# Scalsol/mega.pytorch

Measured on AMD Instinct MI355X. Metric: frames/sec MEGA R-101 inference, 1000x600 VID clip, higher is better.
Workload: dtype bf16

## Files before the change

### mega/pytorch_amd/csrc/spatial.hip

```cpp
#include <cstdlib>

#include "common.h"

namespace {

constexpr int ST_T = 16;
constexpr int ST_P = ST_T * 2 + 5;
constexpr int ST_PW = ST_P + 1;

template <typename OT>
__global__ __launch_bounds__(256) void stem_conv_kernel(const float* __restrict__ in, const float* __restrict__ w,
                                                        const float* __restrict__ scale,
                                                        const float* __restrict__ bias, OT* __restrict__ out, int N,
                                                        int H, int W, int Ho, int Wo) {
  __shared__ float patch[3][ST_P][ST_PW];
  const int tid = threadIdx.x;
  const int n = blockIdx.z;
  const int oy0 = blockIdx.y * ST_T, ox0 = blockIdx.x * ST_T;
  const int iy0 = oy0 * 2 - 3, ix0 = ox0 * 2 - 3;
  for (int e = tid; e < 3 * ST_P * ST_P; e += 256) {
    const int c = e / (ST_P * ST_P);
    const int rem = e - c * ST_P * ST_P;
    const int y = rem / ST_P, x = rem - y * ST_P;
    const int iy = iy0 + y, ix = ix0 + x;
// ... 268 lines not shown
  constexpr int VE = Elem<T>::VE;
  int xo[NC];
#pragma unroll
  for (int c = 0; c < NC; ++c) xo[c] = min(x0 + c, W - 1) * C;
  for (int r = 0; r < NR; r += RU) {
    uint4 rv[RU][NC];
#pragma unroll
    for (int u = 0; u < RU; ++u) {
      const T* rowp = base + (size_t)min(y0 + r + u, H - 1) * W * C;
#pragma unroll
      for (int c = 0; c < NC; ++c) rv[u][c] = *reinterpret_cast<const uint4*>(rowp + xo[c]);
    }
#pragma unroll
    for (int u = 0; u < RU; ++u) {
      const float wyr = r + u < RS_MAXP ? wy[r + u] : 0.f;
#pragma unroll
      for (int c = 0; c < NC; ++c) {
        const T* ev = reinterpret_cast<const T*>(&rv[u][c]);
        const float wgt = wyr * wx[c];
#pragma unroll
        for (int e = 0; e < VE; ++e) acc[e] = fmaf(wgt, Elem<T>::ld(ev + e), acc[e]);
      }
    }
  }
}

template <typename T, int NSLICE, bool PLANES = false, typename PT = bf16_t>
__global__ __launch_bounds__(256, 4) void roi_align_nhwc_sep_kernel(const T* __restrict__ feat,
                                                                 const float* __restrict__ rois, T* __restrict__ out,
                                                                 int K, int C, int H, int W, float spatial_scale,
                                                                 int PH, int PW) {
  static_assert(!PLANES || sizeof(T) == 4, "planes output: f32 features");
  constexpr int VE = Elem<T>::VE;
  auto store = [&](int k_, int bin, int cv, const float (&acc)[Elem<T>::VE], float inv_count) {
    if constexpr (PLANES) {
      float v[4];
#pragma unroll
      for (int e = 0; e < 4; ++e) v[e] = acc[e] * inv_count;
      const unsigned h0 = Half16<PT>::pack2(v[0], v[1]), h1 = Half16<PT>::pack2(v[2], v[3]);
      const unsigned l0 = Half16<PT>::pack2(v[0] - Half16<PT>::lo(h0), v[1] - Half16<PT>::hi(h0));
      const unsigned l1 = Half16<PT>::pack2(v[2] - Half16<PT>::lo(h1), v[3] - Half16<PT>::hi(h1));
      const size_t plane = (size_t)PH * PW * C;
      unsigned short* row = reinterpret_cast<unsigned short*>(out) + (size_t)k_ * 2 * plane + (size_t)bin * C + (size_t)cv * 4;
      *reinterpret_cast<uint2*>(row) = make_uint2(h0, h1);
      *reinterpret_cast<uint2*>(row + plane) = make_uint2(l0, l1);
    } else {
      uint4 o;
      T* oe = reinterpret_cast<T*>(&o);
#pragma unroll
      for (int e = 0; e < VE; ++e) Elem<T>::st(oe + e, acc[e] * inv_count);
      *reinterpret_cast<uint4*>(out + ((size_t)k_ * PH * PW + bin) * C + (size_t)cv * VE) = o;
    }
  };
  __shared__ float s_wy[RS_MAXPW][RS_MAXP + 2];
  __shared__ float s_wx[RS_MAXPW][RS_MAXP];
  __shared__ int s_y[RS_MAXPW][2];
  __shared__ int s_x[RS_MAXPW][2];
  const int CV = C / VE;
  const int slice = NSLICE == 8 ? (int)(blockIdx.x & 7) : 0;
  const int k = NSLICE == 8 ? (int)(blockIdx.x >> 3) : (int)blockIdx.x;
  const int cvs = CV / NSLICE;
  const float* roi = rois + (size_t)k * 5;
  const int b = (int)roi[0];
  const float roi_start_w = roi[1] * spatial_scale;
  const float roi_start_h = roi[2] * spatial_scale;
  const float roi_end_w = roi[3] * spatial_scale;
  const float roi_end_h = roi[4] * spatial_scale;
  const float roi_width = fmaxf(roi_end_w - roi_start_w, 1.f);
  const float roi_height = fmaxf(roi_end_h - roi_start_h, 1.f);
  const float bin_size_h = roi_height / (float)PH;
  const float bin_size_w = roi_width / (float)PW;
  const int grid_h = (int)ceilf(roi_height / (float)PH);
  const int grid_w = (int)ceilf(roi_width / (float)PW);
  const float count = (float)(grid_h * grid_w);
  auto axis = [](float p, int n, int& lo, int& hi, float& wl, float& wh) {
    if (p < -1.0f || p > (float)n) { lo = hi = 0; wl = wh = 0.f; return; }
    if (p <= 0.f) p = 0.f;
    lo = (int)p;
    if (lo >= n - 1) { hi = lo = n - 1; p = (float)lo; } else { hi = lo + 1; }
    wh = p - (float)lo;
    wl = 1.f - wh;
  };
  auto table = [&](float start, float bin_size, int bin_index, int grid, int n, int slot, int& first, int& cnt) {
    int f = n, l = -1;
    for (int i = 0; i < grid; ++i) {
      int lo, hi; float wl, wh;
      axis(start + bin_index * bin_size + (i + .5f) * bin_size / (float)grid, n, lo, hi, wl, wh);
      if (wl + wh > 0.f) { f = min(f, lo); l = max(l, hi); }
    }
    float w = 0.f;
    for (int i = 0; i < grid; ++i) {
      int lo, hi; float wl, wh;
      axis(start + bin_index * bin_size + (i + .5f) * bin_size / (float)grid, n, lo, hi, wl, wh);
      if (wl + wh > 0.f) {
        if (lo - f == slot) w += wl;
        if (hi - f == slot) w += wh;
      }
    }
    if (l < f) { f = 0; l = -1; }
    first = f;
    cnt = l - f + 1;
    return w;
  };
  const int tid = threadIdx.x;
  if (tid < PH * (RS_MAXP + 2)) {
    const int ph = tid / (RS_MAXP + 2), slot = tid - ph * (RS_MAXP + 2);
    int first, cnt;
    const float w = table(roi_start_h, bin_size_h, ph, grid_h, H, slot, first, cnt);
    s_wy[ph][slot] = slot < RS_MAXP ? w : 0.f;
    if (slot == 0) { s_y[ph][0] = first; s_y[ph][1] = cnt; }
  } else if (tid >= 128 && tid < 128 + PW * RS_MAXP) {
    const int pw = (tid - 128) / RS_MAXP, slot = (tid - 128) - pw * RS_MAXP;
    int first, cnt;
    s_wx[pw][slot] = table(roi_start_w, bin_size_w, pw, grid_w, W, slot, first, cnt);
    if (slot == 0) { s_x[pw][0] = first; s_x[pw][1] = cnt; }
  }
  __syncthreads();
  int NR = 0, NCm = 0;
  for (int i = 0; i < PH; ++i) NR = max(NR, s_y[i][1]);
  for (int i = 0; i < PW; ++i) NCm = max(NCm, s_x[i][1]);
  const float inv_count = 1.f / count;
  const T* fb = feat + (size_t)b * H * W * C;
  const int nitem = PH * PW * cvs;
  if (NR > RS_MAXP || NCm > RS_MAXP) {
    for (int item = tid; item < nitem; item += 256) {
      const int bin = item / cvs, ph = bin / PW, pw = bin - ph * PW;
      const int cv = slice * cvs + (item - bin * cvs);
      float acc[VE];
#pragma unroll
      for (int e = 0; e < VE; ++e) acc[e] = 0.f;
      for (int iy = 0; iy < grid_h; ++iy) {
        int ylo, yhi; float wyl, wyh;
        axis(roi_start_h + ph * bin_size_h + (iy + .5f) * bin_size_h / (float)grid_h, H, ylo, yhi, wyl, wyh);
        for (int ix = 0; ix < grid_w; ++ix) {
          int xlo, xhi; float wxl, wxh;
          axis(roi_start_w + pw * bin_size_w + (ix + .5f) * bin_size_w / (float)grid_w, W, xlo, xhi, wxl, wxh);
          if (wyl + wyh == 0.f || wxl + wxh == 0.f) continue;
          const int ys[2] = {ylo, yhi}, xs[2] = {xlo, xhi};
          const float wys[2] = {wyl, wyh}, wxs[2] = {wxl, wxh};
#pragma unroll
          for (int a = 0; a < 2; ++a)
#pragma unroll
            for (int c = 0; c < 2; ++c) {
              const uint4 v = *reinterpret_cast<const uint4*>(fb + ((size_t)ys[a] * W + xs[c]) * C + (size_t)cv * VE);
              const T* ev = reinterpret_cast<const T*>(&v);
              const float wgt = wys[a] * wxs[c];
#pragma unroll
              for (int e = 0; e < VE; ++e) acc[e] = fmaf(wgt, Elem<T>::ld(ev + e), acc[e]);
            }
        }
      }
      store(k, bin, cv, acc, inv_count);
    }
    return;
  }
  for (int item = tid; item < nitem; item += 256) {
    const int bin = item / cvs, ph = bin / PW, pw = bin - ph * PW;
    const int cv = slice * cvs + (item - bin * cvs);
    float acc[VE];
#pragma unroll
    for (int e = 0; e < VE; ++e) acc[e] = 0.f;
    const T* base = fb + (size_t)cv * VE;
    const int y0 = s_y[ph][0], x0 = s_x[pw][0];
    if (NCm <= 3) roi_patch_accumulate<T, 3, 2>(base, W, H, C, y0, x0, NR, s_wy[ph], s_wx[pw], acc);
    else if (NCm <= 4) roi_patch_accumulate<T, 4, 2>(base, W, H, C, y0, x0, NR, s_wy[ph], s_wx[pw], acc);
    else if (NCm <= 6) roi_patch_accumulate<T, 6, 2>(base, W, H, C, y0, x0, NR, s_wy[ph], s_wx[pw], acc);
    else roi_patch_accumulate<T, RS_MAXP, 1>(base, W, H, C, y0, x0, NR, s_wy[ph], s_wx[pw], acc);
    store(k, bin, cv, acc, inv_count);
  }
}

constexpr int SM_TY = 8, SM_TX = 32;
constexpr int SM_PH = 2 * SM_TY + 5, SM_PW = 2 * SM_TX + 5, SM_PS = 72;
constexpr int SM_K = 176, SM_WS = 184;

__host__ __device__ constexpr int stem_group_off(int g) {
  const int gg = g < 21 ? g : 20;
  return (gg / 7) * (SM_PH * SM_PS) + (gg % 7) * SM_PS;
}

template <bool U8>
__global__ __launch_bounds__(256, 4) void stem_mfma_kernel(const void* __restrict__ in_, const bf16_t* __restrict__ w,
                                                        const float* __restrict__ scale,
                                                        const float* __restrict__ bias, bf16_t* __restrict__ out,
                                                        int N, int H, int W, int Ho, int Wo, float m0, float m1, float m2,
                                                        int to_bgr) {
  const float* __restrict__ in = reinterpret_cast<const float*>(in_);
  const unsigned char* __restrict__ in8 = reinterpret_cast<const unsigned char*>(in_);
  constexpr int SM_PATCH_B = (3 * SM_PH * SM_PS * 2 + 15) / 16 * 16, SM_OUT_PS = 144;
  constexpr int SM_LDS_B = SM_TY * SM_TX * SM_OUT_PS > SM_PATCH_B + 64 * SM_WS * 2 ? SM_TY * SM_TX * SM_OUT_PS
                                                                                   : SM_PATCH_B + 64 * SM_WS * 2;
  __shared__ __attribute__((aligned(16))) unsigned char smem[SM_LDS_B];
  unsigned short* patch = reinterpret_cast<unsigned short*>(smem);
  unsigned short* wl = reinterpret_cast<unsigned short*>(smem + SM_PATCH_B);
  const int tid = threadIdx.x, lane = tid & 63, wave = tid >> 6;
  const int n = blockIdx.z;
  const int oy0 = blockIdx.y * SM_TY, ox0 = blockIdx.x * SM_TX;
  const int iy0 = oy0 * 2 - 3, ix0 = ox0 * 2 - 3;
  constexpr int NPL = (3 * SM_PH * SM_PS + 255) / 256, NWL = (64 * (SM_K / 8) + 255) / 256;
  float pv[NPL];
  u32x4_t wv[NWL];
#pragma unroll
  for (int i = 0; i < NPL; ++i) {
    const int e = tid + 256 * i;
    const int c = e / (SM_PH * SM_PS);
    const int rem = e - c * (SM_PH * SM_PS);
    const int y = rem / SM_PS, x = rem - y * SM_PS;
    const int iy = iy0 + y, ix = ix0 + x;
    pv[i] = 0.f;
    if (e < 3 * SM_PH * SM_PS && x < SM_PW && (unsigned)iy < (unsigned)H && (unsigned)ix < (unsigned)W) {
      if (U8) {
        const float mean = c == 0 ? m0 : (c == 1 ? m1 : m2);
        pv[i] = (float)in8[(((size_t)n * H + iy) * W + ix) * 3 + (to_bgr ? 2 - c : c)] - mean;
      } else {
        pv[i] = in[((size_t)(n * 3 + c) * H + iy) * W + ix];
      }
    }
  }
#pragma unroll
  for (int i = 0; i < NWL; ++i) {
    const int e = tid + 256 * i;
    const int row = e / (SM_K / 8), v = e - row * (SM_K / 8);
    if (e < 64 * (SM_K / 8)) wv[i] = *reinterpret_cast<const u32x4_t*>(w + row * SM_K + v * 8);
  }
#pragma unroll
  for (int i = 0; i < NPL; ++i) {
    const int e = tid + 256 * i;
    if (e < 3 * SM_PH * SM_PS) patch[e] = f32_to_bf16(pv[i]);
  }
#pragma unroll
  for (int i = 0; i < NWL; ++i) {
    const int e = tid + 256 * i;
    const int row = e / (SM_K / 8), v = e - row * (SM_K / 8);
    if (e < 64 * (SM_K / 8)) *reinterpret_cast<u32x4_t*>(&wl[row * SM_WS + v * 8]) = wv[i];
  }
  __syncthreads();

  const int p = lane & 31, half = lane >> 5;
  f32x16_t acc[2][2];
#pragma unroll
  for (int i = 0; i < 2; ++i)
#pragma unroll
    for (int j = 0; j < 2; ++j)
#pragma unroll
      for (int r = 0; r < 16; ++r) acc[i][j][r] = 0.f;
#pragma unroll
  for (int ks = 0; ks < SM_K / 16; ++ks) {
    uint4 a[2], b[2];
#pragma unroll
    for (int i = 0; i < 2; ++i) {
      const unsigned* base = reinterpret_cast<const unsigned*>(
          patch + (2 * (2 * wave + i)) * SM_PS + 2 * p + (half ? stem_group_off(2 * ks + 1) : stem_group_off(2 * ks)));
      a[i] = make_uint4(base[0], base[1], base[2], base[3]);
    }
#pragma unroll
    for (int j = 0; j < 2; ++j)
      b[j] = *reinterpret_cast<const uint4*>(&wl[(j * 32 + p) * SM_WS + ks * 16 + half * 8]);
#pragma unroll
    for (int i = 0; i < 2; ++i)
#pragma unroll
      for (int j = 0; j < 2; ++j)
        acc[i][j] = __builtin_amdgcn_mfma_f32_32x32x16_bf16(__builtin_bit_cast(bf16x8_t, a[i]),
                                                            __builtin_bit_cast(bf16x8_t, b[j]), acc[i][j], 0, 0, 0);
  }
  __syncthreads();
#pragma unroll
  for (int j = 0; j < 2; ++j) {
    const int ch = j * 32 + p;
    const float sc = scale[ch], bi = bias[ch];
#pragma unroll
    for (int i = 0; i < 2; ++i) {
#pragma unroll
      for (int r = 0; r < 16; ++r) {
        const int px = (r & 3) + 8 * (r >> 2) + 4 * half;
        *reinterpret_cast<unsigned short*>(smem + ((2 * wave + i) * SM_TX + px) * SM_OUT_PS + ch * 2) =
            (bf16_t)(f32_to_bf16(fmaxf(acc[i][j][r] * sc + bi, 0.f)) & 0x7fffu);
      }
    }
  }
  __syncthreads();
#pragma unroll
  for (int i = 0; i < SM_TY * SM_TX * 8 / 256; ++i) {
    const int v = tid + 256 * i;
    const int pl = v >> 3, cv = v & 7;
    const int oy = oy0 + pl / SM_TX, ox = ox0 + pl % SM_TX;
    if (oy < Ho && ox < Wo)
      *reinterpret_cast<uint4*>(out + (((size_t)n * Ho + oy) * Wo + ox) * 64 + cv * 8) =
          *reinterpret_cast<const uint4*>(smem + pl * SM_OUT_PS + cv * 16);
  }
}

constexpr int SP_PY = 4, SP_PX = 16;
constexpr int SP_TY = 2 * SP_PY + 1, SP_TX = 2 * SP_PX + 1;
constexpr int SP_NPIX = SP_TY * SP_TX;
constexpr int SP_NBLK = (SP_NPIX + 31) / 32;
constexpr int SP_PH = 2 * SP_TY + 5, SP_PW = 2 * SP_TX + 5, SP_PS = 72;
static_assert(SP_PW + 1 <= SP_PS, "the zero-weight 8th tap reads one column past the patch");

__host__ __device__ constexpr int sp_group_off(int g) {
  const int gg = g < 21 ? g : 20;
  return (gg / 7) * (SP_PH * SP_PS) + (gg % 7) * SP_PS;
}

template <bool U8, typename HT = bf16_t>
__global__ __launch_bounds__(256, 3) void stem_pool_kernel(const void* __restrict__ in_, const bf16_t* __restrict__ w,
                                                        const float* __restrict__ scale, const float* __restrict__ bias,
                                                        bf16_t* __restrict__ out, int N, int H, int W, int Ho, int Wo, int Hp,
                                                        int Wp, float m0, float m1, float m2, int to_bgr) {
  const float* __restrict__ in = reinterpret_cast<const float*>(in_);
  const unsigned char* __restrict__ in8 = reinterpret_cast<const unsigned char*>(in_);
  constexpr int PATCH_B = (3 * SP_PH * SP_PS * 2 + 15) / 16 * 16, OUT_PS = 144;
  constexpr int LDS_B = SP_NBLK * 32 * OUT_PS > PATCH_B + 64 * SM_WS * 2 ? SP_NBLK * 32 * OUT_PS : PATCH_B + 64 * SM_WS * 2;
  __shared__ __attribute__((aligned(16))) unsigned char smem[LDS_B];
  unsigned short* patch = reinterpret_cast<unsigned short*>(smem);
  unsigned short* wl = reinterpret_cast<unsigned short*>(smem + PATCH_B);
  const int tid = threadIdx.x, lane = tid & 63, wave = tid >> 6;
  const int n = blockIdx.z;
  const int py0 = blockIdx.y * SP_PY, px0 = blockIdx.x * SP_PX;
  const int oy0 = 2 * py0 - 1, ox0 = 2 * px0 - 1;
  const int iy0 = oy0 * 2 - 3, ix0 = ox0 * 2 - 3;
  constexpr int NPL = (3 * SP_PH * SP_PS + 255) / 256, NWL = (64 * (SM_K / 8) + 255) / 256;
  float pv[NPL];
  u32x4_t wv[NWL];
#pragma unroll
  for (int i = 0; i < NPL; ++i) {
    const int e = tid + 256 * i;
    const int c = e / (SP_PH * SP_PS);
    const int rem = e - c * (SP_PH * SP_PS);
    const int y = rem / SP_PS, x = rem - y * SP_PS;
    const int iy = iy0 + y, ix = ix0 + x;
    pv[i] = 0.f;
    if (e < 3 * SP_PH * SP_PS && x < SP_PW && (unsigned)iy < (unsigned)H && (unsigned)ix < (unsigned)W) {
      if (U8) {
        const float mean = c == 0 ? m0 : (c == 1 ? m1 : m2);
        pv[i] = (float)in8[(((size_t)n * H + iy) * W + ix) * 3 + (to_bgr ? 2 - c : c)] - mean;
      } else {
        pv[i] = in[((size_t)(n * 3 + c) * H + iy) * W + ix];
      }
    }
  }
#pragma unroll
  for (int i = 0; i < NWL; ++i) {
    const int e = tid + 256 * i;
    const int row = e / (SM_K / 8), v = e - row * (SM_K / 8);
    if (e < 64 * (SM_K / 8)) wv[i] = *reinterpret_cast<const u32x4_t*>(w + row * SM_K + v * 8);
  }
#pragma unroll
  for (int i = 0; i < NPL; ++i) {
    const int e = tid + 256 * i;
    if (e < 3 * SP_PH * SP_PS) patch[e] = Half16<HT>::cvt(pv[i]);
  }
#pragma unroll
  for (int i = 0; i < NWL; ++i) {
    const int e = tid + 256 * i;
    const int row = e / (SM_K / 8), v = e - row * (SM_K / 8);
    if (e < 64 * (SM_K / 8)) *reinterpret_cast<u32x4_t*>(&wl[row * SM_WS + v * 8]) = wv[i];
  }
  __syncthreads();

  const int p = lane & 31, half = lane >> 5;
  constexpr int NB = 3;
  f32x16_t acc[NB][2];
  int pbase[NB];
#pragma unroll
  for (int b = 0; b < NB; ++b) {
    const int pix = min(32 * (wave + 4 * b) + p, SP_NPIX - 1);
    const int r = pix / SP_TX, c = pix - r * SP_TX;
    pbase[b] = 2 * r * SP_PS + 2 * c;
#pragma unroll
    for (int j = 0; j < 2; ++j)
#pragma unroll
      for (int q = 0; q < 16; ++q) acc[b][j][q] = 0.f;
  }
#pragma unroll
  for (int ks = 0; ks < SM_K / 16; ++ks) {
    u32x4_t bfr[2];
#pragma unroll
    for (int j = 0; j < 2; ++j) bfr[j] = *reinterpret_cast<const u32x4_t*>(&wl[(j * 32 + p) * SM_WS + ks * 16 + half * 8]);
#pragma unroll
    for (int b = 0; b < NB; ++b) {
      if (wave + 4 * b < SP_NBLK) {
        const unsigned* base = reinterpret_cast<const unsigned*>(patch + pbase[b] + (half ? sp_group_off(2 * ks + 1) : sp_group_off(2 * ks)));
        const u32x4_t a = {base[0], base[1], base[2], base[3]};
#pragma unroll
        for (int j = 0; j < 2; ++j) acc[b][j] = Half16<HT>::mfma32(a, bfr[j], acc[b][j]);
      }
    }
  }
  __syncthreads();
#pragma unroll
  for (int j = 0; j < 2; ++j) {
    const int ch = j * 32 + p;
    const float sc = scale[ch], bi = bias[ch];
#pragma unroll
    for (int b = 0; b < NB; ++b) {
      if (wave + 4 * b < SP_NBLK) {
#pragma unroll
        for (int q = 0; q < 16; ++q) {
          const int pix = 32 * (wave + 4 * b) + (q & 3) + 8 * (q >> 2) + 4 * half;
          const int r = pix / SP_TX, c = pix - r * SP_TX;
          const int oy = oy0 + r, ox = ox0 + c;
          const bool ok = pix < SP_NPIX && (unsigned)oy < (unsigned)Ho && (unsigned)ox < (unsigned)Wo;
          const unsigned short hv = (unsigned short)(Half16<HT>::cvt(fmaxf(acc[b][j][q] * sc + bi, 0.f)) & 0x7fffu);
          *reinterpret_cast<unsigned short*>(smem + pix * OUT_PS + ch * 2) = ok ? hv : (unsigned short)0;
        }
      }
    }
  }
  __syncthreads();
#pragma unroll
  for (int i = 0; i < SP_PY * SP_PX * 8 / 256; ++i) {
    const int v = tid + 256 * i;
    const int pl = v >> 3, cv = v & 7;
    const int ty = pl / SP_PX, tx = pl - ty * SP_PX;
    const int oy = py0 + ty, ox = px0 + tx;
    typedef unsigned short u16x8_t __attribute__((ext_vector_type(8)));
    u16x8_t m = {0, 0, 0, 0, 0, 0, 0, 0};
#pragma unroll
    for (int dy = 0; dy < 3; ++dy)
#pragma unroll
      for (int dx = 0; dx < 3; ++dx) {
        const u16x8_t q = *reinterpret_cast<const u16x8_t*>(smem + ((2 * ty + dy) * SP_TX + 2 * tx + dx) * OUT_PS + cv * 16);
        m = __builtin_elementwise_max(m, q);
      }
    if (oy < Hp && ox < Wp) *reinterpret_cast<u16x8_t*>(out + (((size_t)n * Hp + oy) * Wp + ox) * 64 + cv * 8) = m;
  }
}

}

extern "C" int mega_stem_conv_bn_relu_bf16(const float* in, const void* w_n176_bf16, const float* scale,
                                           const float* bias, void* out, int N, int H, int W, void* stream) {
  mega_clear_error();
  if (!in || !w_n176_bf16 || !scale || !bias || !out || N <= 0 || H <= 0 || W <= 0) return MEGA_ERR_ARG;
  const int Ho = (H + 6 - 7) / 2 + 1, Wo = (W + 6 - 7) / 2 + 1;
  dim3 grid(cdiv(Wo, SM_TX), cdiv(Ho, SM_TY), N);
  hipLaunchKernelGGL(stem_mfma_kernel<false>, grid, dim3(256), 0, (hipStream_t)stream, (const void*)in,
                     (const bf16_t*)w_n176_bf16, scale, bias, (bf16_t*)out, N, H, W, Ho, Wo, 0.f, 0.f, 0.f, 0);
  return mega_check_launch();
}

extern "C" int mega_stem_conv_bn_relu_bf16_u8(const void* frames_u8, const void* w_n176_bf16, const float* scale,
                                              const float* bias, void* out, int N, int H, int W, float mean0, float mean1,
                                              float mean2, int to_bgr, void* stream) {
  mega_clear_error();
  if (!frames_u8 || !w_n176_bf16 || !scale || !bias || !out || N <= 0 || H <= 0 || W <= 0) return MEGA_ERR_ARG;
  const int Ho = (H + 6 - 7) / 2 + 1, Wo = (W + 6 - 7) / 2 + 1;
  dim3 grid(cdiv(Wo, SM_TX), cdiv(Ho, SM_TY), N);
  hipLaunchKernelGGL(stem_mfma_kernel<true>, grid, dim3(256), 0, (hipStream_t)stream, frames_u8, (const bf16_t*)w_n176_bf16,
                     scale, bias, (bf16_t*)out, N, H, W, Ho, Wo, mean0, mean1, mean2, to_bgr);
  return mega_check_launch();
}

extern "C" int mega_stem_conv_bn_relu(const float* in, const float* w_tap64, const float* scale, const float* bias,
                                      void* out, int N, int H, int W, int out_dtype, void* stream) {
  mega_clear_error();
  if (!in || !w_tap64 || !scale || !bias || !out || N <= 0 || H <= 0 || W <= 0) return MEGA_ERR_ARG;
  const int Ho = (H + 6 - 7) / 2 + 1, Wo = (W + 6 - 7) / 2 + 1;
  dim3 grid(cdiv(Wo, ST_T), cdiv(Ho, ST_T), N);
  hipStream_t st = (hipStream_t)stream;
  if (out_dtype == MEGA_BF16)
    hipLaunchKernelGGL((stem_conv_kernel<bf16_t>), grid, dim3(256), 0, st, in, w_tap64, scale, bias, (bf16_t*)out, N, H,
                       W, Ho, Wo);
  else if (out_dtype == MEGA_F32)
    hipLaunchKernelGGL((stem_conv_kernel<float>), grid, dim3(256), 0, st, in, w_tap64, scale, bias, (float*)out, N, H, W,
                       Ho, Wo);
  else
    return MEGA_ERR_ARG;
  return mega_check_launch();
}

extern "C" int mega_maxpool3x3s2_nhwc(const void* in, void* out, int N, int H, int W, int C, int dtype, void* stream) {
  mega_clear_error();
  if (!in || !out || N <= 0 || H <= 0 || W <= 0 || C <= 0) return MEGA_ERR_ARG;
  const int Ho = (H + 2 - 3) / 2 + 1, Wo = (W + 2 - 3) / 2 + 1;
  hipStream_t st = (hipStream_t)stream;
  if (dtype == MEGA_BF16) {
    if (C % 8) return MEGA_ERR_ARG;
    const size_t total = (size_t)N * Ho * Wo * (C / 8);
    const int blocks = (int)((total + 255) / 256 > 8192 ? 8192 : (total + 255) / 256);
    hipLaunchKernelGGL((maxpool_kernel<bf16_t>), dim3(blocks), dim3(256), 0, st, (const bf16_t*)in, (bf16_t*)out, N, H,
                       W, C, Ho, Wo);
  } else if (dtype == MEGA_F16) {
    if (C % 8) return MEGA_ERR_ARG;
    const size_t total = (size_t)N * Ho * Wo * (C / 8);
    const int blocks = (int)((total + 255) / 256 > 8192 ? 8192 : (total + 255) / 256);
    hipLaunchKernelGGL((maxpool_kernel<f16_t>), dim3(blocks), dim3(256), 0, st, (const f16_t*)in, (f16_t*)out, N, H,
                       W, C, Ho, Wo);
  } else if (dtype == MEGA_F32) {
    if (C % 4) return MEGA_ERR_ARG;
    const size_t total = (size_t)N * Ho * Wo * (C / 4);
    const int blocks = (int)((total + 255) / 256 > 8192 ? 8192 : (total + 255) / 256);
    hipLaunchKernelGGL((maxpool_kernel<float>), dim3(blocks), dim3(256), 0, st, (const float*)in, (float*)out, N, H, W,
                       C, Ho, Wo);
  } else {
    return MEGA_ERR_ARG;
  }
  return mega_check_launch();
}

extern "C" int mega_roi_align_fwd(const void* feat, const float* rois, void* out, int K, int C, int H, int W,
                                  float spatial_scale, int pooled_h, int pooled_w, int sampling_ratio, int in_nhwc,
                                  int out_nhwc, int dtype, int out_dtype, void* stream) {
  mega_clear_error();
  if (K == 0) return MEGA_OK;
  if (!feat || !rois || !out || K < 0 || C <= 0 || H <= 0 || W <= 0 || pooled_h <= 0 || pooled_w <= 0)
    return MEGA_ERR_ARG;
  hipStream_t st = (hipStream_t)stream;
  if (in_nhwc && out_nhwc && dtype == out_dtype && C % (dtype != MEGA_F32 ? 8 : 4) == 0) {
    const int CV = C / (dtype != MEGA_F32 ? 8 : 4);
    const long long total = (long long)K * pooled_h * pooled_w * CV;
    static const bool no_slice = getenv("MEGA_ROI_NO_XCD_SLICE") != nullptr;
    const bool sliced = !no_slice && CV % 8 == 0 && CV / 8 >= 16 && total / 8 >= 256 * 64;
    long long nb = ((sliced ? total / 8 : total) + 255) / 256;
    if (nb > 131072) nb = 131072;
    dim3 vgrid((unsigned)(sliced ? nb * 8 : nb));
    static const bool no_sep = getenv("MEGA_ROI_NO_SEPARABLE") != nullptr;
    if (dtype == MEGA_F16 && !no_sep && sampling_ratio <= 0 && pooled_w <= RS_MAXPW && pooled_h <= RS_MAXPW) {
      if (!no_slice && CV % 8 == 0 && CV / 8 >= 16)
        hipLaunchKernelGGL((roi_align_nhwc_sep_kernel<f16_t, 8>), dim3((unsigned)(K * 8)), dim3(256), 0, st,
                           (const f16_t*)feat, rois, (f16_t*)out, K, C, H, W, spatial_scale, pooled_h, pooled_w);
      else
        hipLaunchKernelGGL((roi_align_nhwc_sep_kernel<f16_t, 1>), dim3((unsigned)K), dim3(256), 0, st,
                           (const f16_t*)feat, rois, (f16_t*)out, K, C, H, W, spatial_scale, pooled_h, pooled_w);
      return mega_check_launch();
    }
    if (dtype == MEGA_BF16 && !no_sep && sampling_ratio <= 0 && pooled_w <= RS_MAXPW && pooled_h <= RS_MAXPW) {
      if (!no_slice && CV % 8 == 0 && CV / 8 >= 16)
        hipLaunchKernelGGL((roi_align_nhwc_sep_kernel<bf16_t, 8>), dim3((unsigned)(K * 8)), dim3(256), 0, st,
                           (const bf16_t*)feat, rois, (bf16_t*)out, K, C, H, W, spatial_scale, pooled_h, pooled_w);
      else
        hipLaunchKernelGGL((roi_align_nhwc_sep_kernel<bf16_t, 1>), dim3((unsigned)K), dim3(256), 0, st,
                           (const bf16_t*)feat, rois, (bf16_t*)out, K, C, H, W, spatial_scale, pooled_h, pooled_w);
      return mega_check_launch();
    }
    if (dtype == MEGA_BF16 && sliced)
      hipLaunchKernelGGL((roi_align_nhwc_vec_kernel<bf16_t, true>), vgrid, dim3(256), 0, st, (const bf16_t*)feat, rois,
                         (bf16_t*)out, K, C, H, W, spatial_scale, pooled_h, pooled_w, sampling_ratio);
    else if (dtype == MEGA_BF16)
      hipLaunchKernelGGL((roi_align_nhwc_vec_kernel<bf16_t, false>), vgrid, dim3(256), 0, st, (const bf16_t*)feat, rois,
                         (bf16_t*)out, K, C, H, W, spatial_scale, pooled_h, pooled_w, sampling_ratio);
    else if (dtype == MEGA_F16 && sliced)
      hipLaunchKernelGGL((roi_align_nhwc_vec_kernel<f16_t, true>), vgrid, dim3(256), 0, st, (const f16_t*)feat, rois,
                         (f16_t*)out, K, C, H, W, spatial_scale, pooled_h, pooled_w, sampling_ratio);
    else if (dtype == MEGA_F16)
      hipLaunchKernelGGL((roi_align_nhwc_vec_kernel<f16_t, false>), vgrid, dim3(256), 0, st, (const f16_t*)feat, rois,
                         (f16_t*)out, K, C, H, W, spatial_scale, pooled_h, pooled_w, sampling_ratio);
    else if (dtype == MEGA_F32 && sliced)
      hipLaunchKernelGGL((roi_align_nhwc_vec_kernel<float, true>), vgrid, dim3(256), 0, st, (const float*)feat, rois,
                         (float*)out, K, C, H, W, spatial_scale, pooled_h, pooled_w, sampling_ratio);
    else if (dtype == MEGA_F32)
      hipLaunchKernelGGL((roi_align_nhwc_vec_kernel<float, false>), vgrid, dim3(256), 0, st, (const float*)feat, rois,
                         (float*)out, K, C, H, W, spatial_scale, pooled_h, pooled_w, sampling_ratio);
    else
      return MEGA_ERR_ARG;
    return mega_check_launch();
  }
  dim3 grid((unsigned)(K * pooled_h * pooled_w));
  const int threads = C >= 256 ? 256 : (C >= 128 ? 128 : 64);
  if (dtype == MEGA_BF16 && out_dtype == MEGA_BF16)
    hipLaunchKernelGGL((roi_align_kernel<bf16_t, bf16_t>), grid, dim3(threads), 0, st, (const bf16_t*)feat, rois,
                       (bf16_t*)out, K, C, H, W, spatial_scale, pooled_h, pooled_w, sampling_ratio, in_nhwc, out_nhwc);
  else if (dtype == MEGA_F16 && out_dtype == MEGA_F16)
    hipLaunchKernelGGL((roi_align_kernel<f16_t, f16_t>), grid, dim3(threads), 0, st, (const f16_t*)feat, rois,
                       (f16_t*)out, K, C, H, W, spatial_scale, pooled_h, pooled_w, sampling_ratio, in_nhwc, out_nhwc);
  else if (dtype == MEGA_F32 && out_dtype == MEGA_F32)
    hipLaunchKernelGGL((roi_align_kernel<float, float>), grid, dim3(threads), 0, st, (const float*)feat, rois,
                       (float*)out, K, C, H, W, spatial_scale, pooled_h, pooled_w, sampling_ratio, in_nhwc, out_nhwc);
  else
    return MEGA_ERR_ARG;
  return mega_check_launch();
}

extern "C" int mega_avgpool2x2_ceil_nhwc(const void* in, void* out, int N, int H, int W, int C, int dtype,
                                         void* stream) {
  mega_clear_error();
  if (!in || !out || N <= 0 || H <= 0 || W <= 0 || C <= 0) return MEGA_ERR_ARG;
  const int Ho = (H + 1) / 2, Wo = (W + 1) / 2;
  hipStream_t st = (hipStream_t)stream;
  const int ve = dtype == MEGA_BF16 ? 8 : 4;
  if (C % ve) return MEGA_ERR_ARG;
  const size_t total = (size_t)N * Ho * Wo * (C / ve);
  const int blocks = (int)((total + 255) / 256 > 8192 ? 8192 : (total + 255) / 256);
  if (dtype == MEGA_BF16)
    hipLaunchKernelGGL((avgpool2_kernel<bf16_t>), dim3(blocks), dim3(256), 0, st, (const bf16_t*)in, (bf16_t*)out, N, H,
                       W, C, Ho, Wo);
  else if (dtype == MEGA_F32)
    hipLaunchKernelGGL((avgpool2_kernel<float>), dim3(blocks), dim3(256), 0, st, (const float*)in, (float*)out, N, H, W,
                       C, Ho, Wo);
  else
    return MEGA_ERR_ARG;
  return mega_check_launch();
}

extern "C" int mega_stem_pool_dt(const void* in, int u8, const void* w_n176, const float* scale, const float* bias,
                                 void* out, int N, int H, int W, float mean0, float mean1, float mean2, int to_bgr,
                                 int dtype, void* stream) {
  mega_clear_error();
  if (!in || !w_n176 || !scale || !bias || !out || N <= 0 || H <= 0 || W <= 0) return MEGA_ERR_ARG;
  if (dtype != MEGA_BF16 && dtype != MEGA_F16) return MEGA_ERR_ARG;
  const int Ho = (H + 6 - 7) / 2 + 1, Wo = (W + 6 - 7) / 2 + 1;
  const int Hp = (Ho + 2 - 3) / 2 + 1, Wp = (Wo + 2 - 3) / 2 + 1;
  dim3 grid(cdiv(Wp, SP_PX), cdiv(Hp, SP_PY), N);
  hipStream_t st = (hipStream_t)stream;
  const bf16_t* w = (const bf16_t*)w_n176;
  bf16_t* o = (bf16_t*)out;
  if (!u8) { mean0 = mean1 = mean2 = 0.f; to_bgr = 0; }
  if (dtype == MEGA_F16) {
    if (u8) hipLaunchKernelGGL((stem_pool_kernel<true, f16_t>), grid, dim3(256), 0, st, in, w, scale, bias, o, N, H, W, Ho, Wo, Hp, Wp, mean0, mean1, mean2, to_bgr);
    else hipLaunchKernelGGL((stem_pool_kernel<false, f16_t>), grid, dim3(256), 0, st, in, w, scale, bias, o, N, H, W, Ho, Wo, Hp, Wp, mean0, mean1, mean2, to_bgr);
  } else {
    if (u8) hipLaunchKernelGGL((stem_pool_kernel<true, bf16_t>), grid, dim3(256), 0, st, in, w, scale, bias, o, N, H, W, Ho, Wo, Hp, Wp, mean0, mean1, mean2, to_bgr);
    else hipLaunchKernelGGL((stem_pool_kernel<false, bf16_t>), grid, dim3(256), 0, st, in, w, scale, bias, o, N, H, W, Ho, Wo, Hp, Wp, mean0, mean1, mean2, to_bgr);
  }
  return mega_check_launch();
}

extern "C" int mega_stem_pool_bf16(const void* in, int u8, const void* w_n176_bf16, const float* scale, const float* bias,
                                   void* out, int N, int H, int W, float mean0, float mean1, float mean2, int to_bgr,
                                   void* stream) {
  return mega_stem_pool_dt(in, u8, w_n176_bf16, scale, bias, out, N, H, W, mean0, mean1, mean2, to_bgr, MEGA_BF16, stream);
}

extern "C" int mega_roi_align_fwd_planes_dt(const float* feat, const float* rois, void* out, int K, int C, int H, int W,
                                            float spatial_scale, int pooled_h, int pooled_w, int sampling_ratio, int dtype,
                                            void* stream) {
  mega_clear_error();
  if (K == 0) return MEGA_OK;
  if (dtype != MEGA_BF16 && dtype != MEGA_F16) return MEGA_ERR_ARG;
  if (!feat || !rois || !out || K < 0 || C <= 0 || C % 4 || H <= 0 || W <= 0 || pooled_h <= 0 || pooled_w <= 0) return MEGA_ERR_ARG;
  const int CV = C / 4;
  const long long total = (long long)K * pooled_h * pooled_w * CV;
  const bool sliced = CV % 8 == 0 && CV / 8 >= 16 && total / 8 >= 256 * 64;
  long long nb = ((sliced ? total / 8 : total) + 255) / 256;
  if (nb > 131072) nb = 131072;
  dim3 vgrid((unsigned)(sliced ? nb * 8 : nb));
  hipStream_t st = (hipStream_t)stream;
  static const bool no_sep = getenv("MEGA_ROI_NO_SEPARABLE") != nullptr;
  if (!no_sep && sliced && sampling_ratio <= 0 && pooled_w <= RS_MAXPW && pooled_h <= RS_MAXPW) {
    if (dtype == MEGA_F16)
      hipLaunchKernelGGL((roi_align_nhwc_sep_kernel<float, 8, true, f16_t>), dim3((unsigned)(K * 8)), dim3(256), 0, st, feat, rois,
                         (float*)out, K, C, H, W, spatial_scale, pooled_h, pooled_w);
    else
      hipLaunchKernelGGL((roi_align_nhwc_sep_kernel<float, 8, true, bf16_t>), dim3((unsigned)(K * 8)), dim3(256), 0, st, feat, rois,
                         (float*)out, K, C, H, W, spatial_scale, pooled_h, pooled_w);
    return mega_check_launch();
  }
  if (dtype == MEGA_F16) {
    if (sliced)
      hipLaunchKernelGGL((roi_align_nhwc_vec_kernel<float, true, true, f16_t>), vgrid, dim3(256), 0, st, feat, rois, (float*)out, K, C,
                         H, W, spatial_scale, pooled_h, pooled_w, sampling_ratio);
    else
      hipLaunchKernelGGL((roi_align_nhwc_vec_kernel<float, false, true, f16_t>), vgrid, dim3(256), 0, st, feat, rois, (float*)out, K,
                         C, H, W, spatial_scale, pooled_h, pooled_w, sampling_ratio);
  } else if (sliced)
    hipLaunchKernelGGL((roi_align_nhwc_vec_kernel<float, true, true>), vgrid, dim3(256), 0, st, feat, rois, (float*)out, K, C, H,
                       W, spatial_scale, pooled_h, pooled_w, sampling_ratio);
  else
    hipLaunchKernelGGL((roi_align_nhwc_vec_kernel<float, false, true>), vgrid, dim3(256), 0, st, feat, rois, (float*)out, K, C, H,
                       W, spatial_scale, pooled_h, pooled_w, sampling_ratio);
  return mega_check_launch();
}

extern "C" int mega_roi_align_fwd_planes(const float* feat, const float* rois, void* out, int K, int C, int H, int W,
                                         float spatial_scale, int pooled_h, int pooled_w, int sampling_ratio, void* stream) {
  return mega_roi_align_fwd_planes_dt(feat, rois, out, K, C, H, W, spatial_scale, pooled_h, pooled_w, sampling_ratio, MEGA_BF16,
                                      stream);
}
```

Baseline: 892.4.

## Make stem conv+pool kernel persistent with prefetched next-tile patch loads

```diff
diff --git a/mega/pytorch_amd/csrc/spatial.hip b/mega/pytorch_amd/csrc/spatial.hip
--- a/mega/pytorch_amd/csrc/spatial.hip
+++ b/mega/pytorch_amd/csrc/spatial.hip
@@ -594,128 +594,259 @@
   return (gg / 7) * (SP_PH * SP_PS) + (gg % 7) * SP_PS;
 }
 
+constexpr int SPQ_RD = 54;
+constexpr int SPQ_NU8 = (SP_PH * SPQ_RD + 255) / 256;
+constexpr int SPQ_NF32 = (3 * SP_PH * SP_PS + 255) / 256;
+constexpr int SPQ_PATCH_B = 3 * SP_PH * SP_PS * 2;
+constexpr int SPQ_W_B = 64 * SM_WS * 2;
+constexpr int SPQ_OUT_PS = 144;
+constexpr int SPQ_OUT_B = SP_NPIX * SPQ_OUT_PS;
+constexpr int SPQ_LDS_B = SPQ_PATCH_B + SPQ_W_B + SPQ_OUT_B + 2 * 64 * 4;
+constexpr int SPQ_WG_PER_CU = 2;
+static_assert(SPQ_PATCH_B % 16 == 0 && SPQ_W_B % 16 == 0 && SPQ_OUT_B % 16 == 0, "16-byte aligned LDS areas");
+static_assert(SPQ_WG_PER_CU * SPQ_LDS_B <= 160 * 1024, "two blocks a CU");
+static_assert(SPQ_RD * 4 >= SP_PW * 3 + 3, "a patch row spans at most 216 bytes from its first dword");
+
+#define SPQ_BAR()                                    \
+  do {                                               \
+    asm volatile("s_waitcnt lgkmcnt(0)" ::: "memory"); \
+    __builtin_amdgcn_s_barrier();                    \
+    asm volatile("" ::: "memory");                   \
+  } while (0)
+
+template <int V> struct SpqN { static constexpr int value = V; };
+
+struct SpqTile {
+  int n, py0, px0, iy0, ix0;
+};
+
+__device__ __forceinline__ SpqTile spq_tile(int t, int tiles_x, int tiles_yx) {
+  SpqTile r;
+  r.n = t / tiles_yx;
+  const int rem = t - r.n * tiles_yx;
+  const int ty = rem / tiles_x;
+  r.py0 = ty * SP_PY;
+  r.px0 = (rem - ty * tiles_x) * SP_PX;
+  r.iy0 = 2 * (2 * r.py0 - 1) - 3;
+  r.ix0 = 2 * (2 * r.px0 - 1) - 3;
+  return r;
+}
+
 template <bool U8, typename HT = bf16_t>
-__global__ __launch_bounds__(256, 3) void stem_pool_kernel(const void* __restrict__ in_, const bf16_t* __restrict__ w,
-                                                        const float* __restrict__ scale, const float* __restrict__ bias,
-                                                        bf16_t* __restrict__ out, int N, int H, int W, int Ho, int Wo, int Hp,
-                                                        int Wp, float m0, float m1, float m2, int to_bgr) {
+__global__ __launch_bounds__(256, SPQ_WG_PER_CU) void stem_pool_kernel(const void* __restrict__ in_,
+                                                                     const bf16_t* __restrict__ w,
+                                                                     const float* __restrict__ scale,
+                                                                     const float* __restrict__ bias,
+                                                                     bf16_t* __restrict__ out, int N, int H, int W,
+                                                                     int Ho, int Wo, int Hp, int Wp, float m0, float m1,
+                                                                     float m2, int to_bgr, int tiles_x, int tiles_yx,
+                                                                     int ntiles) {
   const float* __restrict__ in = reinterpret_cast<const float*>(in_);
   const unsigned char* __restrict__ in8 = reinterpret_cast<const unsigned char*>(in_);
-  constexpr int PATCH_B = (3 * SP_PH * SP_PS * 2 + 15) / 16 * 16, OUT_PS = 144;
-  constexpr int LDS_B = SP_NBLK * 32 * OUT_PS > PATCH_B + 64 * SM_WS * 2 ? SP_NBLK * 32 * OUT_PS : PATCH_B + 64 * SM_WS * 2;
-  __shared__ __attribute__((aligned(16))) unsigned char smem[LDS_B];
+  __shared__ __attribute__((aligned(16))) unsigned char smem[SPQ_LDS_B];
   unsigned short* patch = reinterpret_cast<unsigned short*>(smem);
-  unsigned short* wl = reinterpret_cast<unsigned short*>(smem + PATCH_B);
+  unsigned short* wl = reinterpret_cast<unsigned short*>(smem + SPQ_PATCH_B);
+  unsigned char* stg = smem + SPQ_PATCH_B + SPQ_W_B;
+  float* s_sc = reinterpret_cast<float*>(smem + SPQ_PATCH_B + SPQ_W_B + SPQ_OUT_B);
+  float* s_bi = s_sc + 64;
   const int tid = threadIdx.x, lane = tid & 63, wave = tid >> 6;
-  const int n = blockIdx.z;
-  const int py0 = blockIdx.y * SP_PY, px0 = blockIdx.x * SP_PX;
-  const int oy0 = 2 * py0 - 1, ox0 = 2 * px0 - 1;
-  const int iy0 = oy0 * 2 - 3, ix0 = ox0 * 2 - 3;
-  constexpr int NPL = (3 * SP_PH * SP_PS + 255) / 256, NWL = (64 * (SM_K / 8) + 255) / 256;
-  float pv[NPL];
-  u32x4_t wv[NWL];
-#pragma unroll
-  for (int i = 0; i < NPL; ++i) {
-    const int e = tid + 256 * i;
-    const int c = e / (SP_PH * SP_PS);
-    const int rem = e - c * (SP_PH * SP_PS);
-    const int y = rem / SP_PS, x = rem - y * SP_PS;
-    const int iy = iy0 + y, ix = ix0 + x;
-    pv[i] = 0.f;
-    if (e < 3 * SP_PH * SP_PS && x < SP_PW && (unsigned)iy < (unsigned)H && (unsigned)ix < (unsigned)W) {
-      if (U8) {
-        const float mean = c == 0 ? m0 : (c == 1 ? m1 : m2);
-        pv[i] = (float)in8[(((size_t)n * H + iy) * W + ix) * 3 + (to_bgr ? 2 - c : c)] - mean;
-      } else {
-        pv[i] = in[((size_t)(n * 3 + c) * H + iy) * W + ix];
-      }
-    }
-  }
-#pragma unroll
-  for (int i = 0; i < NWL; ++i) {
-    const int e = tid + 256 * i;
-    const int row = e / (SM_K / 8), v = e - row * (SM_K / 8);
-    if (e < 64 * (SM_K / 8)) wv[i] = *reinterpret_cast<const u32x4_t*>(w + row * SM_K + v * 8);
-  }
-#pragma unroll
-  for (int i = 0; i < NPL; ++i) {
-    const int e = tid + 256 * i;
-    if (e < 3 * SP_PH * SP_PS) patch[e] = Half16<HT>::cvt(pv[i]);
-  }
-#pragma unroll
-  for (int i = 0; i < NWL; ++i) {
-    const int e = tid + 256 * i;
-    const int row = e / (SM_K / 8), v = e - row * (SM_K / 8);
-    if (e < 64 * (SM_K / 8)) *reinterpret_cast<u32x4_t*>(&wl[row * SM_WS + v * 8]) = wv[i];
-  }
-  __syncthreads();
+
+  unsigned pd[U8 ? SPQ_NU8 : 1], pt[U8 ? SPQ_NU8 : 1];
+  float pv[U8 ? 1 : SPQ_NF32];
+  auto load_patch = [&](int t) {
+    const SpqTile tl = spq_tile(t, tiles_x, tiles_yx);
+    if constexpr (U8) {
+      const unsigned char* fr = in8 + (size_t)tl.n * H * W * 3;
+      const int fa = (int)(reinterpret_cast<uintptr_t>(fr) & 3);
+      const int nrec = fa + H * W * 3;
+      const __amdgpu_buffer_rsrc_t rs = __builtin_amdgcn_make_buffer_rsrc(const_cast<unsigned char*>(fr - fa), 0, nrec, 0x00020000);
+#pragma unroll
+      for (int i = 0; i < SPQ_NU8; ++i) {
+        const int e = tid + 256 * i;
+        const int y = e / SPQ_RD, d = e - y * SPQ_RD;
+        const int iy = tl.iy0 + y;
+        const int row = fa + iy * W * 3;
+        const int off = ((row + tl.ix0 * 3) & ~3) + 4 * d;
+        const int vlo = row + max(tl.ix0, 0) * 3, vhi = row + min(tl.ix0 + SP_PW, W) * 3;
+        const bool need = e < SP_PH * SPQ_RD && (unsigned)iy < (unsigned)H && off < vhi && off + 4 > vlo;
+        pd[i] = __builtin_amdgcn_raw_buffer_load_b32(rs, need ? (unsigned)off : 0x80000000u, 0, 0);
+        pt[i] = 0;
+      }
+      if (nrec & 3) {
+#pragma unroll
+        for (int i = 0; i < SPQ_NU8; ++i) {
+          const int e = tid + 256 * i;
+          const int y = e / SPQ_RD, d = e - y * SPQ_RD;
+          const int off = ((fa + (tl.iy0 + y) * W * 3 + tl.ix0 * 3) & ~3) + 4 * d;
+          if (e < SP_PH * SPQ_RD && tl.iy0 + y == H - 1 && off < nrec && off + 4 > nrec)
+            for (int b = 0; off + b < nrec; ++b) pt[i] |= (unsigned)fr[off + b - fa] << (8 * b);
+        }
+      }
+    } else {
+      int tid_o = tid;
+      asm volatile("" : "+v"(tid_o));
+#pragma unroll
+      for (int i = 0; i < SPQ_NF32; ++i) {
+        const int e = tid_o + 256 * i;
+        const int c = e / (SP_PH * SP_PS);
+        const int rem = e - c * (SP_PH * SP_PS);
+        const int y = rem / SP_PS, x = rem - y * SP_PS;
+        const int iy = tl.iy0 + y, ix = tl.ix0 + x;
+        pv[i] = 0.f;
+        if (e < 3 * SP_PH * SP_PS && x < SP_PW && (unsigned)iy < (unsigned)H && (unsigned)ix < (unsigned)W)
+          pv[i] = in[((size_t)(tl.n * 3 + c) * H + iy) * W + ix];
+      }
+    }
+  };
+  auto store_patch = [&](int t) {
+    const SpqTile tl = spq_tile(t, tiles_x, tiles_yx);
+    if constexpr (U8) {
+      const float mean0 = m0, mean1 = m1, mean2 = m2;
+      const int fa = (int)((reinterpret_cast<uintptr_t>(in8) + (size_t)tl.n * H * W * 3) & 3);
+#pragma unroll
+      for (int i = 0; i < SPQ_NU8; ++i) {
+        const int e = tid + 256 * i;
+        const int y = e / SPQ_RD, d = e - y * SPQ_RD;
+        const int ye = min(y, SP_PH - 1);
+        const int iy = tl.iy0 + y;
+        const bool row_ok = (unsigned)iy < (unsigned)H;
+        const int s = 4 * d - ((fa + iy * W * 3 + tl.ix0 * 3) & 3);
+        const unsigned v = pd[i] | pt[i];
+#pragma unroll
+        for (int b = 0; b < 4; ++b) {
+          const int o = s + b;
+          const bool in_row = e < SP_PH * SPQ_RD && o >= 0 && o < SP_PW * 3;
+          const int oc = in_row ? o : 0;
+          const int x = oc / 3, ch = oc - 3 * x;
+          const int c = to_bgr ? 2 - ch : ch;
+          const float mean = c == 0 ? mean0 : (c == 1 ? mean1 : mean2);
+          const bool ok = in_row && row_ok && (unsigned)(tl.ix0 + x) < (unsigned)W;
+          const float val = ok ? (float)((v >> (8 * b)) & 255u) - mean : 0.f;
+          patch[in_row ? (c * SP_PH + ye) * SP_PS + x : ye * SP_PS + SP_PS - 1] = Half16<HT>::cvt(val);
+        }
+      }
+    } else {
+#pragma unroll
+      for (int i = 0; i < SPQ_NF32; ++i) {
+        const int e = tid + 256 * i;
+        if (e < 3 * SP_PH * SP_PS) patch[e] = Half16<HT>::cvt(pv[i]);
+      }
+    }
+  };
+
+  {
+    constexpr int NWL = (64 * (SM_K / 8) + 255) / 256;
+    u32x4_t wv[NWL];
+#pragma unroll
+    for (int i = 0; i < NWL; ++i) {
+      const int e = tid + 256 * i;
+      const int row = e / (SM_K / 8), v = e - row * (SM_K / 8);
+      if (e < 64 * (SM_K / 8)) wv[i] = *reinterpret_cast<const u32x4_t*>(w + row * SM_K + v * 8);
+    }
+    float sb = 0.f;
+    if (tid < 128) sb = tid < 64 ? scale[tid] : bias[tid - 64];
+    if (blockIdx.x < ntiles) load_patch(blockIdx.x);
+#pragma unroll
+    for (int i = 0; i < NWL; ++i) {
+      const int e = tid + 256 * i;
+      const int row = e / (SM_K / 8), v = e - row * (SM_K / 8);
+      if (e < 64 * (SM_K / 8)) *reinterpret_cast<u32x4_t*>(&wl[row * SM_WS + v * 8]) = wv[i];
+    }
+    if (tid < 128) s_sc[tid] = sb;
+    if (U8)
+      for (int e = tid; e < 3 * SP_PH; e += 256) patch[e * SP_PS + SP_PS - 1] = 0;
+    if (blockIdx.x < ntiles) store_patch(blockIdx.x);
+    SPQ_BAR();
+  }
 
   const int p = lane & 31, half = lane >> 5;
   constexpr int NB = 3;
-  f32x16_t acc[NB][2];
   int pbase[NB];
 #pragma unroll
   for (int b = 0; b < NB; ++b) {
     const int pix = min(32 * (wave + 4 * b) + p, SP_NPIX - 1);
     const int r = pix / SP_TX, c = pix - r * SP_TX;
     pbase[b] = 2 * r * SP_PS + 2 * c;
-#pragma unroll
-    for (int j = 0; j < 2; ++j)
-#pragma unroll
-      for (int q = 0; q < 16; ++q) acc[b][j][q] = 0.f;
-  }
-#pragma unroll
-  for (int ks = 0; ks < SM_K / 16; ++ks) {
-    u32x4_t bfr[2];
-#pragma unroll
-    for (int j = 0; j < 2; ++j) bfr[j] = *reinterpret_cast<const u32x4_t*>(&wl[(j * 32 + p) * SM_WS + ks * 16 + half * 8]);
+  }
+
+  for (int t = blockIdx.x; t < ntiles; t += gridDim.x) {
+    const int tn = t + gridDim.x;
+    if (U8 && tn < ntiles) load_patch(tn);
+    const SpqTile tl = spq_tile(t, tiles_x, tiles_yx);
+    const int oy0 = 2 * tl.py0 - 1, ox0 = 2 * tl.px0 - 1;
+
+    f32x16_t acc[NB][2];
+#pragma unroll
+    for (int b = 0; b < NB; ++b)
+#pragma unroll
+      for (int j = 0; j < 2; ++j)
+#pragma unroll
+        for (int q = 0; q < 16; ++q) acc[b][j][q] = 0.f;
+    auto mma = [&](auto nbw) {
+#pragma unroll
+      for (int ks = 0; ks < SM_K / 16; ++ks) {
+        u32x4_t wfr[2];
+#pragma unroll
+        for (int j = 0; j < 2; ++j) wfr[j] = *reinterpret_cast<const u32x4_t*>(&wl[(j * 32 + p) * SM_WS + ks * 16 + half * 8]);
+#pragma unroll
+        for (int b = 0; b < decltype(nbw)::value; ++b) {
+          const unsigned* base = reinterpret_cast<const unsigned*>(patch + pbase[b] + (half ? sp_group_off(2 * ks + 1) : sp_group_off(2 * ks)));
+          const u32x4_t a = {base[0], base[1], base[2], base[3]};
+#pragma unroll
+          for (int j = 0; j < 2; ++j) acc[b][j] = Half16<HT>::mfma32(wfr[j], a, acc[b][j]);
+        }
+      }
+    };
+    if (wave + 4 * (NB - 1) < SP_NBLK) mma(SpqN<NB>());
+    else mma(SpqN<NB - 1>());
 #pragma unroll
     for (int b = 0; b < NB; ++b) {
       if (wave + 4 * b < SP_NBLK) {
-        const unsigned* base = reinterpret_cast<const unsigned*>(patch + pbase[b] + (half ? sp_group_off(2 * ks + 1) : sp_group_off(2 * ks)));
-        const u32x4_t a = {base[0], base[1], base[2], base[3]};
-#pragma unroll
-        for (int j = 0; j < 2; ++j) acc[b][j] = Half16<HT>::mfma32(a, bfr[j], acc[b][j]);
-      }
-    }
-  }
-  __syncthreads();
-#pragma unroll
-  for (int j = 0; j < 2; ++j) {
-    const int ch = j * 32 + p;
-    const float sc = scale[ch], bi = bias[ch];
-#pragma unroll
-    for (int b = 0; b < NB; ++b) {
-      if (wave + 4 * b < SP_NBLK) {
-#pragma unroll
-        for (int q = 0; q < 16; ++q) {
-          const int pix = 32 * (wave + 4 * b) + (q & 3) + 8 * (q >> 2) + 4 * half;
-          const int r = pix / SP_TX, c = pix - r * SP_TX;
-          const int oy = oy0 + r, ox = ox0 + c;
-          const bool ok = pix < SP_NPIX && (unsigned)oy < (unsigned)Ho && (unsigned)ox < (unsigned)Wo;
-          const unsigned short hv = (unsigned short)(Half16<HT>::cvt(fmaxf(acc[b][j][q] * sc + bi, 0.f)) & 0x7fffu);
-          *reinterpret_cast<unsigned short*>(smem + pix * OUT_PS + ch * 2) = ok ? hv : (unsigned short)0;
+        const int pix = 32 * (wave + 4 * b) + p;
+        const int r = pix / SP_TX, c = pix - r * SP_TX;
+        const bool ok = (unsigned)(oy0 + r) < (unsigned)Ho && (unsigned)(ox0 + c) < (unsigned)Wo;
+        if (pix < SP_NPIX) {
+#pragma unroll
+          for (int j = 0; j < 2; ++j)
+#pragma unroll
+            for (int g = 0; g < 4; ++g) {
+              const int ch = 32 * j + 8 * g + 4 * half;
+              const f32x4_t sc = *reinterpret_cast<const f32x4_t*>(s_sc + ch);
+              const f32x4_t bi = *reinterpret_cast<const f32x4_t*>(s_bi + ch);
+              unsigned hv[4];
+#pragma unroll
+              for (int q = 0; q < 4; ++q)
+                hv[q] = Half16<HT>::cvt(fmaxf(acc[b][j][4 * g + q] * sc[q] + bi[q], 0.f)) & 0x7fffu;
+              typedef unsigned u32x2_t __attribute__((ext_vector_type(2)));
+              const u32x2_t v2 = {ok ? hv[0] | (hv[1] << 16) : 0u, ok ? hv[2] | (hv[3] << 16) : 0u};
+              *reinterpret_cast<u32x2_t*>(stg + pix * SPQ_OUT_PS + ch * 2) = v2;
+            }
         }
       }
     }
-  }
-  __syncthreads();
-#pragma unroll
-  for (int i = 0; i < SP_PY * SP_PX * 8 / 256; ++i) {
-    const int v = tid + 256 * i;
-    const int pl = v >> 3, cv = v & 7;
-    const int ty = pl / SP_PX, tx = pl - ty * SP_PX;
-    const int oy = py0 + ty, ox = px0 + tx;
-    typedef unsigned short u16x8_t __attribute__((ext_vector_type(8)));
-    u16x8_t m = {0, 0, 0, 0, 0, 0, 0, 0};
-#pragma unroll
-    for (int dy = 0; dy < 3; ++dy)
-#pragma unroll
-      for (int dx = 0; dx < 3; ++dx) {
-        const u16x8_t q = *reinterpret_cast<const u16x8_t*>(smem + ((2 * ty + dy) * SP_TX + 2 * tx + dx) * OUT_PS + cv * 16);
-        m = __builtin_elementwise_max(m, q);
-      }
-    if (oy < Hp && ox < Wp) *reinterpret_cast<u16x8_t*>(out + (((size_t)n * Hp + oy) * Wp + ox) * 64 + cv * 8) = m;
+    SPQ_BAR();
+    if (tn < ntiles) {
+      if (!U8) load_patch(tn);
+      store_patch(tn);
+    }
+#pragma unroll
+    for (int i = 0; i < SP_PY * SP_PX * 8 / 256; ++i) {
+      const int v = tid + 256 * i;
+      const int pl = v >> 3, cv = v & 7;
+      const int ty = pl / SP_PX, tx = pl - ty * SP_PX;
+      const int oy = tl.py0 + ty, ox = tl.px0 + tx;
+      typedef unsigned short u16x8_t __attribute__((ext_vector_type(8)));
+      u16x8_t m = {0, 0, 0, 0, 0, 0, 0, 0};
+#pragma unroll
+      for (int dy = 0; dy < 3; ++dy)
+#pragma unroll
+        for (int dx = 0; dx < 3; ++dx) {
+          const u16x8_t q = *reinterpret_cast<const u16x8_t*>(stg + ((2 * ty + dy) * SP_TX + 2 * tx + dx) * SPQ_OUT_PS + cv * 16);
+          m = __builtin_elementwise_max(m, q);
+        }
+      if (oy < Hp && ox < Wp) *reinterpret_cast<u16x8_t*>(out + (((size_t)tl.n * Hp + oy) * Wp + ox) * 64 + cv * 8) = m;
+    }
+    SPQ_BAR();
   }
 }
 
@@ -893,18 +1024,37 @@
   if (dtype != MEGA_BF16 && dtype != MEGA_F16) return MEGA_ERR_ARG;
   const int Ho = (H + 6 - 7) / 2 + 1, Wo = (W + 6 - 7) / 2 + 1;
   const int Hp = (Ho + 2 - 3) / 2 + 1, Wp = (Wo + 2 - 3) / 2 + 1;
-  dim3 grid(cdiv(Wp, SP_PX), cdiv(Hp, SP_PY), N);
+  const int tiles_x = cdiv(Wp, SP_PX), tiles_yx = cdiv(Hp, SP_PY) * tiles_x;
+  const long tiles = (long)N * tiles_yx;
+  if (tiles > 0x7FFFFFFF || (long)H * W * 3 > 0x7FFFFFFF) return MEGA_ERR_ARG;
+  const int ntiles = (int)tiles;
+  int cus = 256;
+  {
+    static int cached[64] = {0};
+    int dev = 0, n = 0;
+    if (hipGetDevice(&dev) != hipSuccess || dev < 0 || dev >= 64) dev = 0;
+    if (!cached[dev]) {
+      if (hipDeviceGetAttribute(&n, hipDeviceAttributeMultiprocessorCount, dev) == hipSuccess && n > 0) cached[dev] = n;
+      else cached[dev] = 256;
+    }
+    cus = cached[dev];
+  }
+  const dim3 grid(ntiles < SPQ_WG_PER_CU * cus ? ntiles : SPQ_WG_PER_CU * cus);
   hipStream_t st = (hipStream_t)stream;
   const bf16_t* w = (const bf16_t*)w_n176;
   bf16_t* o = (bf16_t*)out;
   if (!u8) { mean0 = mean1 = mean2 = 0.f; to_bgr = 0; }
+#define MEGA_STEM_POOL(U8_, HT_)                                                                                        \
+  hipLaunchKernelGGL((stem_pool_kernel<U8_, HT_>), grid, dim3(256), 0, st, in, w, scale, bias, o, N, H, W, Ho, Wo, Hp, Wp, \
+                     mean0, mean1, mean2, to_bgr, tiles_x, tiles_yx, ntiles)
   if (dtype == MEGA_F16) {
-    if (u8) hipLaunchKernelGGL((stem_pool_kernel<true, f16_t>), grid, dim3(256), 0, st, in, w, scale, bias, o, N, H, W, Ho, Wo, Hp, Wp, mean0, mean1, mean2, to_bgr);
-    else hipLaunchKernelGGL((stem_pool_kernel<false, f16_t>), grid, dim3(256), 0, st, in, w, scale, bias, o, N, H, W, Ho, Wo, Hp, Wp, mean0, mean1, mean2, to_bgr);
+    if (u8) MEGA_STEM_POOL(true, f16_t);
+    else MEGA_STEM_POOL(false, f16_t);
   } else {
-    if (u8) hipLaunchKernelGGL((stem_pool_kernel<true, bf16_t>), grid, dim3(256), 0, st, in, w, scale, bias, o, N, H, W, Ho, Wo, Hp, Wp, mean0, mean1, mean2, to_bgr);
-    else hipLaunchKernelGGL((stem_pool_kernel<false, bf16_t>), grid, dim3(256), 0, st, in, w, scale, bias, o, N, H, W, Ho, Wo, Hp, Wp, mean0, mean1, mean2, to_bgr);
-  }
+    if (u8) MEGA_STEM_POOL(true, bf16_t);
+    else MEGA_STEM_POOL(false, bf16_t);
+  }
+#undef MEGA_STEM_POOL
   return mega_check_launch();
 }
 
```

New measurement: 893.5 (median of 6 runs). Within noise of the previous version (+0.1%).
